# fpthink/EPC-Net

Hardware: AMD Instinct MI355X
Metric: point-clouds/sec (4096 pts) descriptor extraction (higher is better)
Workload: dtype f16x3; 1 GPU; epc-net inference, batch 64x4096x3 fp32 per GPU, NetVLAD K=64, 256-D output (BASELINE.json configs[1]); num_points=4096, precision=EPC_PRECISION_F32 (include/epcnet.h), weights=seeded random init of the architecture (no checkpoint payloads exist), parallelism=independent clouds sharded over 1 GPU(s), no data-path collective

## Files before the change

### epc-net_amd/csrc/head.hip

```cpp
#include "common.h"



template <int GROUPS>
__global__ __launch_bounds__(256) void vlad_fold_kernel(const float* __restrict__ V, const float* __restrict__ colss,
                                                        float* __restrict__ U) {
    constexpr int FPG = 1024 / GROUPS;
    __shared__ float cn[64];
    __shared__ float gsum[64];
    const int slab = blockIdx.x, cloud = blockIdx.y;
    const int k = threadIdx.x & 63, r = threadIdx.x >> 6;
    if (r == 0) {
        float t = 0.f;
#pragma unroll
        for (int g = 0; g < 32; ++g) t += colss[((size_t)cloud * 32 + g) * 64 + k];
        const float inv = 1.0f / sqrtf(fmaxf(t, 1e-12f));
        cn[k] = inv;
        gsum[k] = t * inv * inv;
    }
    __syncthreads();
    float tot = 0.f;
#pragma unroll
    for (int q = 0; q < 64; ++q) tot += gsum[q];
    const float sc = cn[k] * (1.0f / sqrtf(fmaxf(tot, 1e-12f)));
    const float* v = V + (size_t)cloud * 1024 * 64;
    float* uo = U + (size_t)cloud * FPG * 64;
#pragma unroll
    for (int m = 0; m < 4; ++m) {
        const int fi = 16 * slab + r + 4 * m;
        float u = 0.f;
#pragma unroll
        for (int g = 0; g < GROUPS; ++g) u += v[(size_t)(g * FPG + fi) * 64 + k] * sc;
        uo[(size_t)fi * 64 + k] = u;
    }
}

#define HSL 128
__global__ __launch_bounds__(64) void hidden_gemm_kernel(const float* __restrict__ U, const float* __restrict__ H,
                                                         int rows, int kh, float* __restrict__ Yp) {
    const int lane = threadIdx.x, j = lane & 31, h = lane >> 5;
    const int nb = blockIdx.x * 32;
    const int slice = blockIdx.y;
    const int m0 = blockIdx.z * 64;
    const int k0 = slice * HSL;
    f32x16 acc[2];
#pragma unroll
    for (int r = 0; r < 16; ++r) acc[0][r] = acc[1][r] = 0.f;
    const int r0 = m0 + j, r1 = m0 + 32 + j;
    const float* a0p = U + (size_t)min(r0, rows - 1) * kh + k0 + 4 * h;
    const float* a1p = U + (size_t)min(r1, rows - 1) * kh + k0 + 4 * h;
    const float z0 = r0 < rows ? 1.f : 0.f, z1 = r1 < rows ? 1.f : 0.f;
    const float* bp = H + (size_t)(k0 + 4 * h) * 256 + nb + j;
#pragma unroll 8
    for (int q = 0; q < HSL / 8; ++q) {
        const float4 a0 = *reinterpret_cast<const float4*>(a0p + 8 * q);
        const float4 a1 = *reinterpret_cast<const float4*>(a1p + 8 * q);
        const float b0 = bp[(size_t)(8 * q + 0) * 256], b1 = bp[(size_t)(8 * q + 1) * 256];
        const float b2 = bp[(size_t)(8 * q + 2) * 256], b3 = bp[(size_t)(8 * q + 3) * 256];
        acc[0] = mfma32(a0.x * z0, b0, acc[0]);
        acc[1] = mfma32(a1.x * z1, b0, acc[1]);
        acc[0] = mfma32(a0.y * z0, b1, acc[0]);
        acc[1] = mfma32(a1.y * z1, b1, acc[1]);
        acc[0] = mfma32(a0.z * z0, b2, acc[0]);
        acc[1] = mfma32(a1.z * z1, b2, acc[1]);
        acc[0] = mfma32(a0.w * z0, b3, acc[0]);
        acc[1] = mfma32(a1.w * z1, b3, acc[1]);
    }
#pragma unroll
    for (int t = 0; t < 2; ++t)
#pragma unroll
        for (int r = 0; r < 16; ++r) {
            const int row = m0 + 32 * t + mfma_row(r, h);
            if (row < rows) Yp[((size_t)slice * rows + row) * 256 + nb + j] = acc[t][r];
        }
}

__global__ __launch_bounds__(1024) void head_finish_kernel(const float* __restrict__ Yp, int slices, int rows,
                                                           const float* __restrict__ hp, int groups,
                                                           const int32_t* __restrict__ status,
                                                           float* __restrict__ out) {
    __shared__ float part_y[4][256];
    __shared__ float v[256];
    __shared__ float red[4];
    const int cloud = blockIdx.x, c = threadIdx.x & 255, part = threadIdx.x >> 8;
    const float* bn_s = hp;
    const float* bn_t = hp + 256;
    const float* Wg = hp + 512;
    const float* g_s = Wg + 65536;
    const float* g_t = g_s + 256;
    float y = 0.f;
    int s = part;
    for (; s + 28 < slices; s += 32) {
        float t[8];
#pragma unroll
        for (int u = 0; u < 8; ++u) t[u] = Yp[((size_t)(s + 4 * u) * rows + cloud) * 256 + c];
#pragma unroll
        for (int u = 0; u < 8; ++u) y += t[u];
    }
    for (; s < slices; s += 4) y += Yp[((size_t)s * rows + cloud) * 256 + c];
    part_y[part][c] = y;
    __syncthreads();
    const float val = ((part_y[0][c] + part_y[1][c]) + (part_y[2][c] + part_y[3][c])) * bn_s[c] + (float)groups * bn_t[c];
    if (part == 0) v[c] = val;
    __syncthreads();
    float g = 0.f;
#pragma unroll 16
    for (int k = 64 * part; k < 64 * part + 64; ++k) g += v[k] * Wg[k * 256 + c];
    part_y[part][c] = g;
    __syncthreads();
    g = (part_y[0][c] + part_y[1][c]) + (part_y[2][c] + part_y[3][c]);
    g = g * g_s[c] + g_t[c];
    const float o = val * (1.0f / (1.0f + expf(-g)));
    float ss = o * o;
#pragma unroll
    for (int off = 32; off >= 1; off >>= 1) ss += __shfl_xor(ss, off);
    if (part == 0 && (c & 63) == 0) red[c >> 6] = ss;
    __syncthreads();
    const float tot = (red[0] + red[1]) + (red[2] + red[3]);
    const bool poisoned = status && status[cloud] != 0;
    if (part == 0) out[(size_t)cloud * 256 + c] = poisoned ? __int_as_float(0x7fc00000) : o * (1.0f / sqrtf(fmaxf(tot, 1e-12f)));
}

__global__ __launch_bounds__(1024) void fc_head_kernel(const float* __restrict__ pooled,
                                                       const float* __restrict__ pack,
                                                       const int32_t* __restrict__ status, float* __restrict__ out) {
    __shared__ float m[1024];
    __shared__ float part_y[4][256];
    __shared__ float red[4];
    const int cloud = blockIdx.x, c = threadIdx.x & 255, part = threadIdx.x >> 8;
    m[threadIdx.x] = pooled[(size_t)cloud * 1024 + threadIdx.x];
    __syncthreads();
    float y = 0.f;
#pragma unroll 16
    for (int k = 256 * part; k < 256 * part + 256; ++k) y += m[k] * pack[k * 256 + c];
    part_y[part][c] = y;
    __syncthreads();
    y = fmaxf(((part_y[0][c] + part_y[1][c]) + (part_y[2][c] + part_y[3][c])) + pack[1024 * 256 + c], 0.f);
    float ss = y * y;
#pragma unroll
    for (int off = 32; off >= 1; off >>= 1) ss += __shfl_xor(ss, off);
    if (part == 0 && (c & 63) == 0) red[c >> 6] = ss;
    __syncthreads();
    const float tot = (red[0] + red[1]) + (red[2] + red[3]);
    const bool poisoned = status && status[cloud] != 0;
    if (part == 0) out[(size_t)cloud * 256 + c] = poisoned ? __int_as_float(0x7fc00000) : y * (1.0f / sqrtf(fmaxf(tot, 1e-12f)));
}

static inline size_t align_up(size_t v, size_t a) { return (v + a - 1) / a * a; }

extern "C" size_t epc_vlad_head_workspace_bytes(int num_clouds, int groups) {
    if (num_clouds <= 0 || groups <= 0 || 64 % groups) return 0;
    const size_t kh = 65536 / groups;
    const size_t u = align_up((size_t)num_clouds * kh * sizeof(float), 256);
    const size_t yp = align_up((kh / HSL) * (size_t)num_clouds * 256 * sizeof(float), 256);
    return u + yp;
}

extern "C" int epc_vlad_head_fwd(const float* V, const float* colss, const void* packed_head, int groups,
                                 int num_clouds, float* out, const int32_t* status, void* workspace,
                                 size_t workspace_bytes, void* stream) {
    EPC_CHECK_ARG(V && colss && packed_head && out && workspace, "null pointer");
    EPC_CHECK_ARG(groups > 0 && 64 % groups == 0, "GROUPS must divide 64");
    EPC_CHECK_ARG(num_clouds >= 0, "bad shape");
    if (num_clouds == 0) return EPC_OK;
    if (workspace_bytes < epc_vlad_head_workspace_bytes(num_clouds, groups)) {
        epc_set_error("epc_vlad_head_fwd: workspace too small");
        return EPC_ENOMEM;
    }
    const int kh = 65536 / groups;
    const float* hp = (const float*)packed_head;
    const float* Hw = hp + 65536;
    const float* tail = Hw + (size_t)kh * 256;
    char* wsp = (char*)workspace;
    float* U = (float*)wsp;
    wsp += align_up((size_t)num_clouds * kh * sizeof(float), 256);
    float* Yp = (float*)wsp;
    hipStream_t st = (hipStream_t)stream;
    EPC_CHECK_ARG(num_clouds <= 65535, "too many clouds per call");
    switch (groups) {
#define EPC_VF(G)                                                                                                  \
    case G:                                                                                                        \
        hipLaunchKernelGGL(vlad_fold_kernel<G>, dim3(1024 / G / 16, num_clouds), dim3(256), 0, st, V, colss, U);   \
        break;
        EPC_VF(1) EPC_VF(2) EPC_VF(4) EPC_VF(8) EPC_VF(16)
#undef EPC_VF
        default:
            epc_set_error("epc_vlad_head_fwd: GROUPS must be one of 1,2,4,8,16");
            return EPC_EINVAL;
    }
    EPC_CHECK_LAUNCH();
    const int slices = kh / HSL;
    hipLaunchKernelGGL(hidden_gemm_kernel, dim3(8, slices, (num_clouds + 63) / 64), dim3(64), 0, st, U, Hw,
                       num_clouds, kh, Yp);
    EPC_CHECK_LAUNCH();
    hipLaunchKernelGGL(head_finish_kernel, dim3(num_clouds), dim3(1024), 0, st, Yp, slices, num_clouds, tail,
                       groups, status, out);
    EPC_CHECK_LAUNCH();
    return EPC_OK;
}

extern "C" int epc_fc_head_fwd(const float* pooled, const void* packed_fc, int num_clouds, float* out,
                               const int32_t* status, void* stream) {
    EPC_CHECK_ARG(pooled && packed_fc && out, "null pointer");
    EPC_CHECK_ARG(num_clouds >= 0, "bad shape");
    if (num_clouds == 0) return EPC_OK;
    hipLaunchKernelGGL(fc_head_kernel, dim3(num_clouds), dim3(1024), 0, (hipStream_t)stream, pooled,
                       (const float*)packed_fc, status, out);
    EPC_CHECK_LAUNCH();
    return EPC_OK;
}
```

Measured before the change: 59070 clouds/s.

## Restructure hidden GEMM with 4-wave split-K, LDS-staged loads, prefetched weights

The hidden-layer GEMM moves from 64-thread blocks over 128-wide K slices to 256-thread blocks over 512-wide slices. Each wave takes a quarter of the slice, prefetches its U and H tiles into registers, and transposes U through LDS so the global loads coalesce. The four wave partials are then reduced in LDS before store, which cuts the number of slice partials written to Yp and summed later. The finish kernel also preloads its gating weights and per-channel scales into registers before the first barrier, hiding their latency behind the Yp reduction. The cost is heavier register and LDS use per block and fewer blocks in the grid.

```diff
diff --git a/epc-net_amd/csrc/head.hip b/epc-net_amd/csrc/head.hip
--- a/epc-net_amd/csrc/head.hip
+++ b/epc-net_amd/csrc/head.hip
@@ -35,44 +35,68 @@
     }
 }
 
-#define HSL 128
-__global__ __launch_bounds__(64) void hidden_gemm_kernel(const float* __restrict__ U, const float* __restrict__ H,
-                                                         int rows, int kh, float* __restrict__ Yp) {
-    const int lane = threadIdx.x, j = lane & 31, h = lane >> 5;
-    const int nb = blockIdx.x * 32;
-    const int slice = blockIdx.y;
+#define HSL 512
+__global__ __launch_bounds__(256) void hidden_gemm_kernel(const float* __restrict__ U, const float* __restrict__ H,
+                                                          int rows, int kh, float* __restrict__ Yp) {
+    constexpr int KW = HSL / 4, NCH = KW / 32;
+    constexpr int SROW = 36;
+    constexpr int STAGE = 64 * SROW, RED = 32 * 64;
+    __shared__ __attribute__((aligned(16))) float lds[4 * (STAGE > RED ? STAGE : RED)];
+    const int lane = threadIdx.x & 63, w = threadIdx.x >> 6, j = lane & 31, h = lane >> 5;
+    const int slice = blockIdx.x;
+    const int nb = blockIdx.y * 32;
     const int m0 = blockIdx.z * 64;
-    const int k0 = slice * HSL;
+    const int k0 = slice * HSL + w * KW;
+    const int lr = lane >> 3, lk = 4 * (lane & 7);
+    float4 ul[NCH][8];
+    float hb[NCH][16];
+#pragma unroll
+    for (int ch = 0; ch < NCH; ++ch) {
+#pragma unroll
+        for (int i = 0; i < 8; ++i)
+            ul[ch][i] = ld4(U + (size_t)min(m0 + 8 * i + lr, rows - 1) * kh + k0 + 32 * ch + lk);
+#pragma unroll
+        for (int s = 0; s < 16; ++s) hb[ch][s] = H[(size_t)(k0 + 32 * ch + 8 * (s >> 2) + 4 * h + (s & 3)) * 256 + nb + j];
+    }
     f32x16 acc[2];
 #pragma unroll
     for (int r = 0; r < 16; ++r) acc[0][r] = acc[1][r] = 0.f;
-    const int r0 = m0 + j, r1 = m0 + 32 + j;
-    const float* a0p = U + (size_t)min(r0, rows - 1) * kh + k0 + 4 * h;
-    const float* a1p = U + (size_t)min(r1, rows - 1) * kh + k0 + 4 * h;
-    const float z0 = r0 < rows ? 1.f : 0.f, z1 = r1 < rows ? 1.f : 0.f;
-    const float* bp = H + (size_t)(k0 + 4 * h) * 256 + nb + j;
-#pragma unroll 8
-    for (int q = 0; q < HSL / 8; ++q) {
-        const float4 a0 = *reinterpret_cast<const float4*>(a0p + 8 * q);
-        const float4 a1 = *reinterpret_cast<const float4*>(a1p + 8 * q);
-        const float b0 = bp[(size_t)(8 * q + 0) * 256], b1 = bp[(size_t)(8 * q + 1) * 256];
-        const float b2 = bp[(size_t)(8 * q + 2) * 256], b3 = bp[(size_t)(8 * q + 3) * 256];
-        acc[0] = mfma32(a0.x * z0, b0, acc[0]);
-        acc[1] = mfma32(a1.x * z1, b0, acc[1]);
-        acc[0] = mfma32(a0.y * z0, b1, acc[0]);
-        acc[1] = mfma32(a1.y * z1, b1, acc[1]);
-        acc[0] = mfma32(a0.z * z0, b2, acc[0]);
-        acc[1] = mfma32(a1.z * z1, b2, acc[1]);
-        acc[0] = mfma32(a0.w * z0, b3, acc[0]);
-        acc[1] = mfma32(a1.w * z1, b3, acc[1]);
-    }
+    float* st = lds + w * STAGE;
+#pragma unroll
+    for (int ch = 0; ch < NCH; ++ch) {
+#pragma unroll
+        for (int i = 0; i < 8; ++i) st4(st + (8 * i + lr) * SROW + lk, ul[ch][i]);
+        __builtin_amdgcn_fence(__ATOMIC_ACQ_REL, "wavefront");
+        float a[2][4][4];
+#pragma unroll
+        for (int t = 0; t < 2; ++t)
+#pragma unroll
+            for (int q = 0; q < 4; ++q) {
+                const float4 v = ld4(st + (32 * t + j) * SROW + 8 * q + 4 * h);
+                a[t][q][0] = v.x, a[t][q][1] = v.y, a[t][q][2] = v.z, a[t][q][3] = v.w;
+            }
+        __builtin_amdgcn_fence(__ATOMIC_ACQ_REL, "wavefront");
+#pragma unroll
+        for (int s = 0; s < 16; ++s)
+#pragma unroll
+            for (int t = 0; t < 2; ++t) acc[t] = mfma32(a[t][s >> 2][s & 3], hb[ch][s], acc[t]);
+    }
+    __syncthreads();
+    float* red = lds + w * RED;
 #pragma unroll
     for (int t = 0; t < 2; ++t)
 #pragma unroll
-        for (int r = 0; r < 16; ++r) {
-            const int row = m0 + 32 * t + mfma_row(r, h);
-            if (row < rows) Yp[((size_t)slice * rows + row) * 256 + nb + j] = acc[t][r];
-        }
+        for (int r = 0; r < 16; ++r) red[(t * 16 + r) * 64 + lane] = acc[t][r];
+    __syncthreads();
+    const int t = w >> 1;
+#pragma unroll
+    for (int i = 0; i < 8; ++i) {
+        const int r = 8 * (w & 1) + i;
+        const int row = m0 + 32 * t + mfma_row(r, h);
+        const float* p = lds + (t * 16 + r) * 64 + lane;
+        const float v = (p[0] + p[RED]) + (p[2 * RED] + p[3 * RED]);
+        if (row < rows) Yp[((size_t)slice * rows + row) * 256 + nb + j] = v;
+    }
 }
 
 __global__ __launch_bounds__(1024) void head_finish_kernel(const float* __restrict__ Yp, int slices, int rows,
@@ -88,6 +112,11 @@
     const float* Wg = hp + 512;
     const float* g_s = Wg + 65536;
     const float* g_t = g_s + 256;
+    float wg[64];
+#pragma unroll
+    for (int k = 0; k < 64; ++k) wg[k] = Wg[(64 * part + k) * 256 + c];
+    const float bs = bn_s[c], bt = bn_t[c], gs = g_s[c], gt = g_t[c];
+    const bool poisoned = status && status[cloud] != 0;
     float y = 0.f;
     int s = part;
     for (; s + 28 < slices; s += 32) {
@@ -100,16 +129,16 @@
     for (; s < slices; s += 4) y += Yp[((size_t)s * rows + cloud) * 256 + c];
     part_y[part][c] = y;
     __syncthreads();
-    const float val = ((part_y[0][c] + part_y[1][c]) + (part_y[2][c] + part_y[3][c])) * bn_s[c] + (float)groups * bn_t[c];
+    const float val = ((part_y[0][c] + part_y[1][c]) + (part_y[2][c] + part_y[3][c])) * bs + (float)groups * bt;
     if (part == 0) v[c] = val;
     __syncthreads();
     float g = 0.f;
-#pragma unroll 16
-    for (int k = 64 * part; k < 64 * part + 64; ++k) g += v[k] * Wg[k * 256 + c];
+#pragma unroll
+    for (int k = 0; k < 64; ++k) g += v[64 * part + k] * wg[k];
     part_y[part][c] = g;
     __syncthreads();
     g = (part_y[0][c] + part_y[1][c]) + (part_y[2][c] + part_y[3][c]);
-    g = g * g_s[c] + g_t[c];
+    g = g * gs + gt;
     const float o = val * (1.0f / (1.0f + expf(-g)));
     float ss = o * o;
 #pragma unroll
@@ -117,7 +146,6 @@
     if (part == 0 && (c & 63) == 0) red[c >> 6] = ss;
     __syncthreads();
     const float tot = (red[0] + red[1]) + (red[2] + red[3]);
-    const bool poisoned = status && status[cloud] != 0;
     if (part == 0) out[(size_t)cloud * 256 + c] = poisoned ? __int_as_float(0x7fc00000) : o * (1.0f / sqrtf(fmaxf(tot, 1e-12f)));
 }
 
@@ -190,8 +218,8 @@
     }
     EPC_CHECK_LAUNCH();
     const int slices = kh / HSL;
-    hipLaunchKernelGGL(hidden_gemm_kernel, dim3(8, slices, (num_clouds + 63) / 64), dim3(64), 0, st, U, Hw,
-                       num_clouds, kh, Yp);
+    hipLaunchKernelGGL(hidden_gemm_kernel, dim3(slices, 8, (num_clouds + 63) / 64), dim3(256), 0, st, U, Hw, num_clouds, kh,
+                       Yp);
     EPC_CHECK_LAUNCH();
     hipLaunchKernelGGL(head_finish_kernel, dim3(num_clouds), dim3(1024), 0, st, Yp, slices, num_clouds, tail,
                        groups, status, out);
```

New measurement: 59480 clouds/s, median of 6. About the same (+0.7%).
